# VinAIResearch/GeoFormer

Hardware: AMD Instinct MI355X
Metric: scenes/sec forward (ScanNetV2 ~150k pts) (higher is better)
Workload: dtype f32

## Files before the change

### geoformer_amd/csrc/mask_head.hip

```cpp
#include "common.h"

#ifndef MH_Q
#define MH_Q 2
#endif
#ifndef MH_MINB
#define MH_MINB 3
#endif

__device__ __forceinline__ float mh_xor32(float v, int lane) {
    const auto r = __builtin_amdgcn_permlane32_swap(__float_as_uint(v), __float_as_uint(v), false, false);
    return __uint_as_float(lane < 32 ? r[1] : r[0]);
}
__device__ __forceinline__ float mh_xor16(float v, int lane) {
    const auto r = __builtin_amdgcn_permlane16_swap(__float_as_uint(v), __float_as_uint(v), false, false);
    return __uint_as_float((lane & 16) ? r[0] : r[1]);
}

__device__ __forceinline__ float mh_relu(float x) { return __int_as_float(max(__float_as_int(x), 0)); }

typedef short bf16x4 __attribute__((ext_vector_type(4)));
typedef short mh_s8 __attribute__((ext_vector_type(8)));
typedef __bf16 mh_bf16x8 __attribute__((ext_vector_type(8)));
__device__ __forceinline__ f32x4 mh_mfma2(bf16x4 a1, bf16x4 a2, bf16x4 b1, bf16x4 b2, f32x4 acc) {
    const mh_s8 a = __builtin_shufflevector(a1, a2, 0, 1, 2, 3, 4, 5, 6, 7), b = __builtin_shufflevector(b1, b2, 0, 1, 2, 3, 4, 5, 6, 7);
    return __builtin_amdgcn_mfma_f32_16x16x32_bf16(__builtin_bit_cast(mh_bf16x8, a), __builtin_bit_cast(mh_bf16x8, b), acc, 0, 0, 0);
}
__device__ __forceinline__ void mh_split3(float x, unsigned& h, unsigned& m, unsigned& l) {
    const unsigned hb = __float_as_uint(x) & 0xffff0000u;
    const float r1 = x - __uint_as_float(hb);
    const unsigned mb = __float_as_uint(r1) & 0xffff0000u;
    const float r2 = r1 - __uint_as_float(mb);
    h = hb >> 16;
    m = mb >> 16;
    l = __float_as_uint(r2) >> 16;
}
__device__ __forceinline__ void mh_split3x4(const float (&x)[4], bf16x4& h, bf16x4& m, bf16x4& l) {
#pragma unroll
    for (int s = 0; s < 4; s++) {
        unsigned a, b, c;
        mh_split3(x[s], a, b, c);
        h[s] = (short)a;
        m[s] = (short)b;
        l[s] = (short)c;
    }
}
__global__ void k_mh_split(const float* __restrict__ feat, int n16, unsigned short* __restrict__ fs) {
    const int i = blockIdx.x * blockDim.x + threadIdx.x;
    if (i >= n16) return;
    unsigned h, m, l;
    mh_split3(feat[i], h, m, l);
    fs[i] = (unsigned short)h;
    fs[(size_t)n16 + i] = (unsigned short)m;
    fs[2 * (size_t)n16 + i] = (unsigned short)l;
}

template <bool USE_GEO, bool SPLIT, bool TINY>
__global__ __launch_bounds__(256, MH_MINB) void k_mask_head(const float* __restrict__ feat, const float* __restrict__ coords,
                                                      const float* __restrict__ geo, const float* __restrict__ qxyz,
                                                      const float* __restrict__ mx, const float* __restrict__ w1,
                                                      const float* __restrict__ b1, const float* __restrict__ w2,
                                                      const float* __restrict__ b2, int ldp, int N, int nq, int qmod,
                                                      int chunks, const unsigned short* __restrict__ fs,
                                                      float* __restrict__ out) {
    const int ld_w1 = ldp ? ldp : 16 * 19, ld_v = ldp ? ldp : 16, ld_s = ldp ? ldp : 1;
    const int lane = threadIdx.x & 63, g = lane >> 4, j = lane & 15;
    const int wave = (blockIdx.x * blockDim.x + threadIdx.x) >> 6;
    const int qgroups = (nq + MH_Q - 1) / MH_Q;
    const int qg = wave % qgroups, chunk = wave / qgroups;
    if (chunk >= chunks) return;
    const int nblocks = (N + 63) >> 6;
    const int per = (nblocks + chunks - 1) / chunks;
    const int blk0 = chunk * per, blk1 = min(nblocks, blk0 + per);

    float wf[MH_Q][4];
    float w5[MH_Q];
    float ww[MH_Q][4], b2q[MH_Q], qc[MH_Q], mq[MH_Q];
#pragma unroll
    for (int t = 0; t < MH_Q; t++) {
        const int q = min(qg * MH_Q + t, nq - 1);
        const float* W = w1 + (size_t)q * ld_w1;
#pragma unroll
        for (int s = 0; s < 4; s++) wf[t][s] = W[j * 19 + 3 + 4 * g + s];
        w5[t] = g < 3 ? W[j * 19 + g] : b1[(size_t)q * ld_v + j];
#pragma unroll
        for (int r = 0; r < 4; r++) ww[t][r] = w2[(size_t)q * ld_v + 4 * g + r];
        b2q[t] = b2[(size_t)q * ld_s];
        const int qs = q % qmod;
        qc[t] = g < 3 ? qxyz[qs * 3 + g] : 1.f;
        mq[t] = (USE_GEO && g < 3) ? mx[qs] : 0.f;
    }
    bf16x4 wh[MH_Q], wm[MH_Q], wl[MH_Q];
    if constexpr (SPLIT) {
#pragma unroll
        for (int t = 0; t < MH_Q; t++) mh_split3x4(wf[t], wh[t], wm[t], wl[t]);
    }
    int qrow[MH_Q];
#pragma unroll
    for (int u = 0; u < MH_Q; u++) qrow[u] = min(qg * MH_Q + u, nq - 1) % qmod;

    struct Block {
        float4 f[4];
        bf16x4 fh[4], fm[4], fl[4];
        float pc[4];
        float gd[MH_Q][4];
    };
    const size_t n16 = (size_t)N * 16;
    auto fetch = [&](int blk, Block& B) {
        const int p0 = TINY ? blk * 64 : min(blk * 64, N - 64);
#pragma unroll
        for (int t = 0; t < 4; t++) {
            const int pc = TINY ? min(p0 + 16 * t + j, N - 1) : p0 + 16 * t + j;
            if constexpr (SPLIT) {
                const size_t e = (size_t)pc * 16 + 4 * g;
                B.fh[t] = *reinterpret_cast<const bf16x4*>(fs + e);
                B.fm[t] = *reinterpret_cast<const bf16x4*>(fs + n16 + e);
                B.fl[t] = *reinterpret_cast<const bf16x4*>(fs + 2 * n16 + e);
            } else {
                B.f[t] = *reinterpret_cast<const float4*>(feat + (size_t)pc * 16 + 4 * g);
            }
            B.pc[t] = g < 3 ? coords[(size_t)pc * 3 + g] : 0.f;
#pragma unroll
            for (int u = 0; u < MH_Q; u++)
                B.gd[u][t] = USE_GEO ? geo[(size_t)qrow[u] * N + pc] : 0.f;
        }
    };
    auto compute = [&](const Block& cur, int blk) {
        const int p0 = TINY ? blk * 64 : min(blk * 64, N - 64);
#pragma unroll
        for (int t = 0; t < MH_Q; t++) {
            const int q = qg * MH_Q + t;
            float part[4];
#pragma unroll
            for (int tl = 0; tl < 4; tl++) {
                float rel = qc[t] - cur.pc[tl];
                if (USE_GEO) {
                    const float ms = __uint_as_float((__float_as_uint(rel) & 0x80000000u) | __float_as_uint(mq[t]));
                    rel = rel + ((cur.gd[t][tl] < 0.f && rel != 0.f) ? ms : 0.f);
                }
                f32x4 acc = {0.f, 0.f, 0.f, 0.f};
                acc = __builtin_amdgcn_mfma_f32_16x16x4f32(w5[t], rel, acc, 0, 0, 0);
                if constexpr (SPLIT) {
                    acc = mh_mfma2(wl[t], wh[t], cur.fh[tl], cur.fl[tl], acc);
                    acc = mh_mfma2(wm[t], wm[t], cur.fm[tl], cur.fh[tl], acc);
                    acc = mh_mfma2(wh[t], wh[t], cur.fm[tl], cur.fh[tl], acc);
                } else {
                    acc = __builtin_amdgcn_mfma_f32_16x16x4f32(wf[t][0], cur.f[tl].x, acc, 0, 0, 0);
                    acc = __builtin_amdgcn_mfma_f32_16x16x4f32(wf[t][1], cur.f[tl].y, acc, 0, 0, 0);
                    acc = __builtin_amdgcn_mfma_f32_16x16x4f32(wf[t][2], cur.f[tl].z, acc, 0, 0, 0);
                    acc = __builtin_amdgcn_mfma_f32_16x16x4f32(wf[t][3], cur.f[tl].w, acc, 0, 0, 0);
                }
                float s = 0.f;
#pragma unroll
                for (int r = 0; r < 4; r++) s = fmaf(ww[t][r], mh_relu(acc[r]), s);
                part[tl] = s;
            }
            {
                const bool hi = g >= 2;
                const float send0 = hi ? part[0] : part[2], send1 = hi ? part[1] : part[3];
                const float r0 = mh_xor32(send0, lane), r1 = mh_xor32(send1, lane);
                const float k0 = (hi ? part[2] : part[0]) + r0, k1 = (hi ? part[3] : part[1]) + r1;
                const bool odd = g & 1;
                const float send = odd ? k0 : k1;
                const float r = mh_xor16(send, lane);
                const float tot = (odd ? k1 : k0) + r + b2q[t];
                const int p = p0 + 16 * g + j;
                if (p < N && q < nq) out[(size_t)q * N + p] = tot;
            }
        }
    };
    Block bufA, bufB;
    if (blk0 < blk1) fetch(blk0, bufA);
    for (int blk = blk0; blk < blk1; blk += 2) {
        if (blk + 1 < blk1) fetch(blk + 1, bufB);
        compute(bufA, blk);
        if (blk + 1 < blk1) {
            if (blk + 2 < blk1) fetch(blk + 2, bufA);
            compute(bufB, blk + 1);
        }
    }
}

extern "C" int gf_mask_head_packed(const float* feat, const float* coords, const float* geo, const float* qxyz,
                                   const float* sqrt_max_geo, const float* w1, const float* b1, const float* w2,
                                   const float* b2, int ldp, int N, int nq, int C, float* out, void* stream);
extern "C" int gf_mask_head_episodes(const float* feat, const float* coords, const float* geo, const float* qxyz,
                                     const float* sqrt_max_geo, const float* w1, const float* b1, const float* w2,
                                     const float* b2, int ldp, int N, int nq, int E, int C, void* split_ws, float* out,
                                     void* stream);
extern "C" size_t gf_mask_head_split_bytes(int N) { return (size_t)(N > 0 ? N : 0) * 16 * 3 * sizeof(unsigned short); }
extern "C" int gf_mask_head(const float* feat, const float* coords, const float* geo, const float* qxyz,
                            const float* sqrt_max_geo, const float* w1, const float* b1, const float* w2,
                            const float* b2, int N, int nq, int C, float* out, void* stream) {
    return gf_mask_head_packed(feat, coords, geo, qxyz, sqrt_max_geo, w1, b1, w2, b2, 0, N, nq, C, out, stream);
}

extern "C" int gf_mask_head_packed(const float* feat, const float* coords, const float* geo, const float* qxyz,
                                   const float* sqrt_max_geo, const float* w1, const float* b1, const float* w2,
                                   const float* b2, int ldp, int N, int nq, int C, float* out, void* stream) {
    return gf_mask_head_episodes(feat, coords, geo, qxyz, sqrt_max_geo, w1, b1, w2, b2, ldp, N, nq, 1, C, nullptr, out, stream);
}

extern "C" int gf_mask_head_episodes(const float* feat, const float* coords, const float* geo, const float* qxyz,
                                     const float* sqrt_max_geo, const float* w1, const float* b1, const float* w2,
                                     const float* b2, int ldp, int N, int nq_scene, int E, int C, void* split_ws, float* out,
                                     void* stream) {
    GF_CHECK_ARG(ldp >= 0, "gf_mask_head: negative parameter stride");
    GF_CHECK_ARG(C == 16, "gf_mask_head: only the 16-channel mask head (m=16) is implemented, got C=%d", C);
    GF_CHECK_ARG(N >= 0 && nq_scene >= 0 && E >= 1, "gf_mask_head: bad sizes");
    GF_CHECK_ARG((long long)nq_scene * E < (1ll << 30), "gf_mask_head: %d episodes x %d queries", E, nq_scene);
    GF_CHECK_ARG((geo == nullptr) == (sqrt_max_geo == nullptr), "gf_mask_head: geo and sqrt_max_geo come together");
    if (N == 0 || nq_scene == 0) return GF_OK;
    const int qmod = nq_scene, nq = nq_scene * E;
    const int qgroups = (nq + MH_Q - 1) / MH_Q;
    const int nblocks = (N + 63) / 64;
    int chunks = (256 * 4 * 8 + qgroups - 1) / qgroups;
    if (chunks > nblocks) chunks = nblocks;
    if (chunks < 1) chunks = 1;
    const long long waves = (long long)qgroups * chunks;
    dim3 grid((unsigned)((waves + 3) / 4));
    hipStream_t st = (hipStream_t)stream;
    const unsigned short* fs = (const unsigned short*)split_ws;
    if (fs) {
        GF_CHECK_ARG(((uintptr_t)fs % 8) == 0, "gf_mask_head: split_ws must be 8-byte aligned");
        const int n16 = N * 16;
        hipLaunchKernelGGL(k_mh_split, dim3(gf_div_up(n16, 256)), dim3(256), 0, st, feat, n16, (unsigned short*)split_ws);
    }
#define MH_LAUNCH(GEO_, SPLIT_)                                                                                          \
    do {                                                                                                                 \
        if (N < 64)                                                                                                      \
            GF_LAUNCH_OP(GF_OP_MASK_HEAD, (k_mask_head<GEO_, SPLIT_, true>), grid, dim3(256), 0, st, feat, coords, geo, qxyz, \
                         sqrt_max_geo, w1, b1, w2, b2, ldp, N, nq, qmod, chunks, fs, out);                               \
        else                                                                                                             \
            GF_LAUNCH_OP(GF_OP_MASK_HEAD, (k_mask_head<GEO_, SPLIT_, false>), grid, dim3(256), 0, st, feat, coords, geo, qxyz, \
                         sqrt_max_geo, w1, b1, w2, b2, ldp, N, nq, qmod, chunks, fs, out);                               \
    } while (0)
    if (geo && fs) MH_LAUNCH(true, true);
    else if (geo) MH_LAUNCH(true, false);
    else if (fs) MH_LAUNCH(false, true);
    else MH_LAUNCH(false, false);
#undef MH_LAUNCH
    GF_CHECK_LAUNCH("gf_mask_head");
    return GF_OK;
}

#define MHB_Q 4

template <bool USE_GEO>
__global__ __launch_bounds__(256, 2) void k_mask_head_bwd_feat(const float* __restrict__ feat, const float* __restrict__ coords,
                                                               const float* __restrict__ geo, const float* __restrict__ qxyz,
                                                               const float* __restrict__ mx, const float* __restrict__ w1,
                                                               const float* __restrict__ b1, const float* __restrict__ w2,
                                                               const float* __restrict__ gout, int ldp, int N, int nq,
                                                               int qmod, int qsplit, float* __restrict__ dfeat) {
    const int ld_w1 = ldp ? ldp : 16 * 19, ld_v = ldp ? ldp : 16;
    const int lane = threadIdx.x & 63, g = lane >> 4, j = lane & 15;
    const int wave = (blockIdx.x * blockDim.x + threadIdx.x) >> 6;
    const int nblocks = (N + 63) >> 6;
    const int blk = wave / qsplit, part = wave - blk * qsplit;
// ... 255 lines not shown
```

### geoformer_amd/model/geoformer.py

```python
from __future__ import annotations

import functools
import os

import numpy as np
import torch
import torch.nn as nn
from torch.nn import functional as F

from .. import _lib, pointops, spconv, unet_exec, unet_train
from . import config as _config
from .backbone import ResidualBlock, UBlock, conv1d_bn_relu, random_downsample
from .layers import (BatchNorm1d, BigLinear, GenericMLP, LazyRelPos, PointwiseConv1d, PositionEmbeddingCoordsSine, RelPosSpec,
                     TransformerDecoder,
                     TransformerDecoderLayer, scene_counts)
from .set_abstraction import PointnetSAModuleVotesSeparate


class _Voxelization(torch.autograd.Function):

    @staticmethod
    def forward(ctx, feats, map_rule, mode=4):
        ctx.rule, ctx.mode, ctx.N = map_rule, mode, feats.shape[0]
        return pointops.voxelize_fp(feats.contiguous(), map_rule, mode)
# ... 800 lines not shown
    def mask_heads_forward(self, geo_dist, mask_features, weights, biases, num_insts, coords_, fps_sampling_coords,
                           use_geo=True):
        n_mask = mask_features.size(0)
        if (mask_features.is_cuda and self.output_dim == 16 and not torch.is_grad_enabled()):
            mx = None
            if use_geo:
                early = self._early()
                hit = next((early.pop(k) for k in list(early) if k[0] == "mx" and early[k][0] is geo_dist), None)
                if hit is not None:
                    torch.cuda.current_stream().wait_event(hit[2])
                    mx = hit[1]
                else:
                    mx = torch.max(geo_dist, dim=1)[0]
                    mx = torch.sqrt(torch.where(mx < 0, torch.max(mx), mx)).contiguous()
            od = self.output_dim
            logits = pointops.mask_head(
                mask_features.reshape(n_mask, od).contiguous(), coords_.contiguous(),
                geo_dist.contiguous() if use_geo else None, fps_sampling_coords.reshape(-1, 3).contiguous(), mx,
                weights[0].reshape(num_insts, od, od + 3).contiguous(), biases[0].reshape(num_insts, od).contiguous(),
                weights[1].reshape(num_insts, od).contiguous(), biases[1].reshape(num_insts).contiguous())
            return logits.reshape(1, num_insts, n_mask)
        rel = fps_sampling_coords.reshape(-1, 1, 3) - coords_.reshape(1, -1, 3)
        if use_geo:
            mx = torch.max(geo_dist, dim=1)[0]
            mx = torch.sqrt(torch.where(mx < 0, torch.max(mx), mx))
            rel = torch.where((geo_dist < 0).unsqueeze(-1), rel + mx[:, None, None] * torch.sign(rel), rel)
        w1, w2 = weights[0].reshape(num_insts, self.output_dim, -1), weights[1].reshape(num_insts, 1, -1)
        b1, b2 = biases[0].reshape(num_insts, self.output_dim, 1), biases[1].reshape(num_insts, 1, 1)
        feat = mask_features.reshape(n_mask, -1)
        h = torch.matmul(w1[:, :, :3], rel.permute(0, 2, 1)) + torch.matmul(w1[:, :, 3:], feat.t().unsqueeze(0)) + b1
        x = torch.matmul(w2, F.relu(h)) + b2
        return x.reshape(1, num_insts, n_mask)

    def _mask_head_packed(self, geo_dist, mask_features, params, num_insts, coords_, fps_sampling_coords):
        n_mask = mask_features.size(0)
        early = self._early()
        hit = next((early.pop(k) for k in list(early) if k[0] == "mx" and early[k][0] is geo_dist), None)
        if hit is not None:
            torch.cuda.current_stream().wait_event(hit[2])
            mx = hit[1]
        else:
            mx = torch.max(geo_dist, dim=1)[0]
            mx = torch.sqrt(torch.where(mx < 0, torch.max(mx), mx)).contiguous()
        logits = pointops.mask_head_packed(mask_features.reshape(n_mask, self.output_dim).contiguous(),
                                           coords_.contiguous(), geo_dist.contiguous(),
                                           fps_sampling_coords.reshape(-1, 3).contiguous(), mx, params.contiguous())
        return logits.reshape(1, num_insts, n_mask)

    def get_mask_prediction(self, geo_dists, param_kernels, mask_features, locs_float_, fps_sampling_locs,
                            batch_offsets_):
        num_layers, n_queries, batch = param_kernels.shape[:3]
        offs = _offsets_list(batch_offsets_)
        outputs = []
        fused_train = (mask_features.is_cuda and torch.is_grad_enabled() and self.output_dim == 16 and self.use_coords
                       and os.environ.get("GF_FUSED_BWD", "1") != "0")
        per_scene, train_ctrl = {}, {}
        if fused_train:
            for b in range(batch):
                s, e = offs[b], offs[b + 1]
                if e - s == 0:
                    continue
                g = geo_dists[b].contiguous()
                mx = torch.max(g, dim=1)[0]
                mx = torch.sqrt(torch.where(mx < 0, torch.max(mx), mx)).contiguous()
                per_scene[b] = (mask_features[s:e].reshape(e - s, self.output_dim).contiguous(),
                                locs_float_[s:e].contiguous(), g, fps_sampling_locs[b].reshape(-1, 3).contiguous(), mx)
        for l, pk in enumerate(param_kernels.unbind(0) if fused_train else param_kernels):
            pk2 = pk.transpose(0, 1).flatten(0, 1)
            sem_chain = self._pointwise_chain("detr_sem_head", [self.detr_sem_head], pk2)
            tow_chain = self._pointwise_chain("before_embedding_tower", [self.before_embedding_tower], pk2)
            packed = False
            if sem_chain is not None and tow_chain is not None:
                rows = pk2.contiguous()
                packed = self.output_dim == 16 and self.use_coords
                cls_done = None
                if packed and rows.is_cuda and not torch.is_grad_enabled() and batch == 1 and not pointops.co_resident():
                    main = torch.cuda.current_stream(rows.device)
                    aux = _SIDE_STREAMS.get((rows.device, main.cuda_stream, "aux"))
                    if aux is not None:
                        rows_ready = torch.cuda.Event()
                        rows_ready.record(main)
                        aux.wait_event(rows_ready)
                        with torch.cuda.stream(aux):
                            cls_logits = pointops.pointwise_mlp(rows, sem_chain).reshape(batch, n_queries, -1)
                            cls_done = torch.cuda.Event()
                            cls_done.record(aux)
                        rows.record_stream(aux)
                        cls_logits.record_stream(main)
                if cls_done is None:
                    cls_logits = pointops.pointwise_mlp(rows, sem_chain).reshape(batch, n_queries, -1)
                emb = pointops.pointwise_mlp(rows, tow_chain)
                controllers = F.linear(emb, self.controller.weight[:, :, 0], self.controller.bias)
            else:
                cls_logits = self.detr_sem_head(pk.permute(1, 2, 0)).transpose(1, 2)
                controllers = self.controller(self.before_embedding_tower(pk2.unsqueeze(2))).squeeze(2)
            controllers = controllers.reshape(batch, n_queries, -1)
            ctrl = controllers.unbind(0) if fused_train else controllers
            mask_logits_list = []
            for b in range(batch):
                s, e = offs[b], offs[b + 1]
                if e - s == 0:
                    mask_logits_list.append(None)
                    continue
                if packed and mask_features.is_cuda and not torch.is_grad_enabled():
                    ml = self._mask_head_packed(geo_dists[b], mask_features[s:e], controllers[b], n_queries,
                                                locs_float_[s:e], fps_sampling_locs[b])
                elif fused_train:
                    train_ctrl.setdefault(b, []).append(ctrl[b])
                    mask_logits_list.append(None)
                    continue
                else:
                    weights, biases = self.parse_dynamic_params(controllers[b], self.output_dim)
                    ml = self.mask_heads_forward(geo_dists[b], mask_features[s:e], weights, biases, n_queries,
                                                 locs_float_[s:e], fps_sampling_locs[b], use_geo=self.use_coords)
                mask_logits_list.append(ml.squeeze(0))
            if packed and cls_done is not None:
                torch.cuda.current_stream(cls_logits.device).wait_event(cls_done)
            outputs.append({"cls_logits": cls_logits, "mask_logits": mask_logits_list})
        for b, ctrls in train_ctrl.items():
            mf_b, locs_b, g, fps_b, mx = per_scene[b]
            logits = pointops.mask_head_train_episodes(mf_b, torch.stack(ctrls), locs_b, g, fps_b, mx)
            for l, ml in enumerate(logits.unbind(0)):
                outputs[l]["mask_logits"][b] = ml
        return outputs

    def generate_proposal(self, mask_logits, cls_logits, fg_idxs, batch_offsets, batch_offsets_,
                          semantic_scores_=None, logit_thresh=0.5, score_thresh=0.5, npoint_thresh=100, sem_prob=None,
                          defer=False, knn_flags=(), segments=None):
        b = 0
        segments = None if torch.is_grad_enabled() else _segments_arg(segments)
        if mask_logits[b].is_cuda and not torch.is_grad_enabled():
            offs, offs_ = _offsets_list(batch_offsets), _offsets_list(batch_offsets_)
            num_points = int(offs[b + 1] - offs[b])
            logits = mask_logits[b].contiguous()
            if sem_prob is not None and isinstance(sem_prob, tuple):
                sem_t = sem_prob[1][:, offs_[b]:offs_[b + 1]]
            else:
                sem = sem_prob if sem_prob is not None else F.softmax(semantic_scores_, dim=1)
                sem_t = sem[offs_[b]:offs_[b + 1]].t()
# ... 152 lines not shown
        if len(fg_idxs) == 0:
            if agree is not None:
                agree(False, locs_float.device)
            outputs["mask_predictions"] = None
            if all_scenes:
                empty = [([], [], []) for _ in range(batch_size)]
                outputs["proposal_scores_per_scene"] = PendingBatchProposals(batch_size, value=empty) \
                    if defer_proposals else empty
            return outputs
        if not fused_fg:
            batch_idxs_ = batch_idxs[fg_idxs]
            locs_float_ = locs_float[fg_idxs]
            output_feats_ = pointops.take_rows_unique(output_feats, fg_idxs)
            semantic_scores_ = semantic_scores[fg_idxs]
        batch_offsets_ = get_batch_offsets(batch_idxs_, batch_size, host_only=fused_fg and not training)
        offs_ = _offsets_list(batch_offsets_)
        nonempty = min(offs_[b + 1] - offs_[b] for b in range(batch_size)) > 0
        n_scenes, scene_ids = batch_size, list(range(batch_size))
        if all_scenes and not nonempty:
            scene_ids = [b for b in range(batch_size) if offs_[b + 1] > offs_[b]]
            offs_ = [offs_[b] for b in scene_ids] + [offs_[-1]]
            batch_offsets_ = torch.tensor(offs_, dtype=torch.int32, device=batch_offsets_.device)
            pc_dims = [pc_dims[0][scene_ids], pc_dims[1][scene_ids]]
            batch_size, nonempty = len(scene_ids), True
        if agree is not None and not agree(nonempty, locs_float.device):
            outputs["mask_predictions"] = None
            return outputs

        def sampling_independent(graphs_only=None):
            if graphs_only is True:
                return knn_graphs(locs_float_, batch_offsets_, batch_size, neighbor=64, radius=0.05)
            chain = self._pointwise_chain("mask_tower", [self.mask_tower], output_feats_)
            if chain is not None:
                mf = pointops.pointwise_mlp(output_feats_.contiguous(), chain).unsqueeze(2)
            else:
                mf = self._mask_tower_rows(output_feats_)
                if mf is None:
                    mf = self.mask_tower(output_feats_.unsqueeze(2).permute(2, 1, 0)).permute(2, 1, 0)
            sp = None
            if not training:
                sp = F.softmax(semantic_scores_, dim=1)
                if sp.is_cuda:
                    sp = (sp, sp.t().contiguous())
            if graphs_only is False:
                return mf, sp
            gr = None
            if locs_float_.is_cuda and nonempty:
                gr = knn_graphs(locs_float_, batch_offsets_, batch_size, neighbor=64, radius=0.05)
            return mf, sp, gr

        max_step = 128 if self.training else 256
        geo_dists = None
        overlap = locs_float_.is_cuda and nonempty and os.environ.get("GF_OVERLAP", "1") != "0"
        if overlap and fused_fg and not training:
            contexts, geo_dists, (mask_features_, sem_prob, graphs) = self._aggregate_geodesic_overlapped(
                locs_float_, output_feats_, batch_offsets_, batch_size, None, max_step, pc_dims, epilogue=True,
                early=sampling_independent, presampled=presampled if fused_fg else None,
                presampled_before=draw_bufs["before"] if (fused_fg and presampled is not None) else None)
        else:
            mask_features_, sem_prob, graphs = sampling_independent()
            if graphs is not None and overlap:
                contexts, geo_dists = self._aggregate_geodesic_overlapped(locs_float_, output_feats_, batch_offsets_,
                                                                          batch_size, graphs, max_step, pc_dims,
                                                                          epilogue=not torch.is_grad_enabled())
            else:
                contexts = self.forward_aggregator(locs_float_, output_feats_, batch_offsets_, batch_size)
        if contexts is None:
# ... 61 lines not shown
```

### geoformer_amd/pointops.py

```python
from __future__ import annotations

import contextlib
import os
import threading

import numpy as np
import torch

from . import _abi, _lib
from ._lib import check, ptr, stream_ptr


def _f32c(t, name):
    if not (t.is_cuda and t.dtype == torch.float32 and t.is_contiguous()):
        raise RuntimeError(f"{name}: expected a contiguous float32 tensor on the GPU")
    return t


def _i32c(t, name):
    if not (t.is_cuda and t.dtype == torch.int32 and t.is_contiguous()):
        raise RuntimeError(f"{name}: expected a contiguous int32 tensor on the GPU")
    return t


# ... 341 lines not shown
        dev = torch.device(device)
        idx = dev.index if dev.index is not None else torch.cuda.current_device()
    for key in list(_SCRATCH):
        if device is None or key[0] == idx:
            del _SCRATCH[key]


def scratch_bytes():
    return sum(t.numel() * t.element_size() for t in _SCRATCH.values() if t is not None)


def geodesic_bfs(D, I, deg, src, radius, max_step, wg_threads=1024):
    _f32c(D, "D"); _i32c(I, "I"); _i32c(src, "src")
    n, K = D.shape
    nq = src.shape[0]
    dev = D.device
    geo = torch.empty((nq, n), dtype=torch.float32, device=dev)
    lib = _lib.load()
    keys = scratch("bfs_keys", nq * n, torch.int64, dev)
    qwords = int(lib.gf_geodesic_bfs_queue_words(n))
    queues = scratch("bfs_queues", nq * qwords, torch.int32, dev)
    check(lib.gf_geodesic_bfs_cfg(ptr(D), ptr(I), ptr(deg), n, K, ptr(src), nq, float(radius), int(max_step),
                                          ptr(geo), ptr(keys), ptr(queues), qwords, int(wg_threads), stream_ptr()),
          "gf_geodesic_bfs")
    return geo


def _mask_head_split_ws(N, device, split):
    if not split:
        return None
    return scratch("mask_head_split", _lib.load().gf_mask_head_split_bytes(N) // 8 + 1, torch.int64, device)


def mask_head(feat, coords, geo, qxyz, sqrt_max_geo, w1, b1, w2, b2, split=True):
    for t, name in ((feat, "feat"), (coords, "coords"), (qxyz, "qxyz"), (w1, "w1"), (b1, "b1"), (w2, "w2"), (b2, "b2")):
        _f32c(t, name)
    N, C = feat.shape
    nq = qxyz.shape[0]
    out = torch.empty((nq, N), dtype=torch.float32, device=feat.device)
    check(_lib.load().gf_mask_head_episodes(ptr(feat), ptr(coords), ptr(geo), ptr(qxyz), ptr(sqrt_max_geo), ptr(w1), ptr(b1),
                                            ptr(w2), ptr(b2), 0, N, nq, 1, C, ptr(_mask_head_split_ws(N, feat.device, split)),
                                            ptr(out), stream_ptr()), "gf_mask_head")
    return out


def mask_head_packed(feat, coords, geo, qxyz, sqrt_max_geo, params, split=True):
    return mask_head_episodes(feat, coords, geo, qxyz, sqrt_max_geo, params.unsqueeze(0), split=split)[0]


def mask_head_episodes(feat, coords, geo, qxyz, sqrt_max_geo, params, split=True):
    for t, name in ((feat, "feat"), (coords, "coords"), (qxyz, "qxyz"), (params, "params")):
        _f32c(t, name)
    N, C = feat.shape
    E, nq, ld = params.shape
    if ld != C * (C + 3) + C + C + 1 or qxyz.shape[0] != nq:
        raise RuntimeError(f"mask_head_episodes: params {tuple(params.shape)} for {qxyz.shape[0]} queries, C={C}")
    base = params.data_ptr()
    o_w2, o_b1, o_b2 = C * (C + 3), C * (C + 3) + C, C * (C + 3) + 2 * C
    out = torch.empty((E, nq, N), dtype=torch.float32, device=feat.device)
    check(_lib.load().gf_mask_head_episodes(ptr(feat), ptr(coords), ptr(geo), ptr(qxyz), ptr(sqrt_max_geo), base,
                                            base + 4 * o_b1, base + 4 * o_w2, base + 4 * o_b2, ld, N, nq, E, C,
                                            ptr(_mask_head_split_ws(N, feat.device, split)), ptr(out), stream_ptr()),
          "gf_mask_head_episodes")
    return out


class _MaskHeadFn(torch.autograd.Function):

    @staticmethod
    def forward(ctx, feat, params, coords, geo, qxyz, sqrt_max_geo):
        ctx.save_for_backward(feat, params, coords, geo, qxyz, sqrt_max_geo)
        return mask_head_packed(feat, coords, geo, qxyz, sqrt_max_geo, params)

    @staticmethod
    def backward(ctx, gout):
        feat, params, coords, geo, qxyz, mx = ctx.saved_tensors
        N, C = feat.shape
        nq, ld = params.shape
        lib = _lib.load()
        dparams = torch.empty_like(params)
        dfeat = torch.zeros_like(feat)
        scratch = torch.empty(lib.gf_mask_head_bwd_scratch_floats(N, nq), dtype=torch.float32, device=feat.device)
        base = params.data_ptr()
        o_w2, o_b1 = C * (C + 3), C * (C + 3) + C
        check(lib.gf_mask_head_bwd(ptr(feat), ptr(coords), ptr(geo), ptr(qxyz), ptr(mx), base, base + 4 * o_b1,
                                   base + 4 * o_w2, ptr(gout.contiguous()), ld, N, nq, C, ptr(dparams), ptr(dfeat),
                                   ptr(scratch), stream_ptr()), "gf_mask_head_bwd")
        return dfeat, dparams, None, None, None, None


class _MaskHeadEpisodesFn(torch.autograd.Function):

    @staticmethod
    def forward(ctx, feat, params, coords, geo, qxyz, sqrt_max_geo):
        ctx.save_for_backward(feat, params, coords, geo, qxyz, sqrt_max_geo)
# ... 1421 lines not shown
```

### include/geoformer_hip.h

```cpp
#ifndef GEOFORMER_HIP_H
#define GEOFORMER_HIP_H

#include <stddef.h>
#include <stdint.h>

#ifdef __cplusplus
extern "C" {
#endif

#define GF_ABI_VERSION 7

typedef enum {
    GF_OK = 0,
    GF_ERR_INVALID_ARG = -1,
    GF_ERR_LAUNCH = -2,
    GF_ERR_UNSUPPORTED = -3,
    GF_ERR_CALLBACK = -4,
} gf_status;

int gf_abi_version(void);
const char* gf_last_error(void);

size_t gf_fg_scratch_bytes(int N);
int gf_fg_select(const float* scores, int N, int C, int cls, int mode, const float* locs, const int32_t* batch_idxs,
// ... 192 lines not shown
int gf_group_points_grad(const float* grad_out, const int32_t* idx, int b, int c, int n, int npoints, int nsample,
                         float* grad_points, void* stream);
int gf_ball_query(const float* new_xyz, const float* xyz, int b, int n, int m, float radius, int nsample, int32_t* idx,
                  void* stream);
size_t gf_fps_scratch_bytes(int b);
int gf_furthest_point_sampling(const float* xyz, int b, int n, int m, int32_t* idxs, void* scratch, void* stream);
const int32_t* gf_fps_error_flag(void* scratch, int b);
int gf_furthest_point_sampling_resume(const float* xyz, int b, int n, int m, int m_known, int32_t* idxs,
                                      void* scratch, void* stream);


size_t gf_knn_scratch_bytes(int n);
int gf_knn_radius(const float* xyz, int n, int k, float radius, int sqrt_out, float* D, int32_t* I, int32_t* deg,
                  void* scratch, void* stream);
const int32_t* gf_knn_error_flag(void* scratch, int n);

size_t gf_geodesic_bfs_queue_words(int n);
int gf_geodesic_bfs(const float* D, const int32_t* I, const int32_t* deg, int n, int K, const int32_t* src, int nq,
                    float radius, int max_step, float* geo, void* keys_ws, void* queue_ws, void* stream);
int gf_geodesic_bfs_cfg(const float* D, const int32_t* I, const int32_t* deg, int n, int K, const int32_t* src, int nq,
                        float radius, int max_step, float* geo, void* keys_ws, void* queue_ws, size_t queue_words,
                        int wg_threads, void* stream);

int gf_mask_head(const float* feat, const float* coords, const float* geo, const float* qxyz,
                 const float* sqrt_max_geo, const float* w1, const float* b1, const float* w2, const float* b2, int N,
                 int nq, int C, float* out, void* stream);
int gf_mask_head_packed(const float* feat, const float* coords, const float* geo, const float* qxyz,
                        const float* sqrt_max_geo, const float* w1, const float* b1, const float* w2, const float* b2,
                        int ldp, int N, int nq, int C, float* out, void* stream);
size_t gf_mask_head_split_bytes(int N);
int gf_mask_head_episodes(const float* feat, const float* coords, const float* geo, const float* qxyz,
                          const float* sqrt_max_geo, const float* w1, const float* b1, const float* w2, const float* b2,
                          int ldp, int N, int nq, int E, int C, void* split_ws, float* out, void* stream);

size_t gf_mask_head_bwd_scratch_floats(int N, int nq);
int gf_mask_head_bwd(const float* feat, const float* coords, const float* geo, const float* qxyz,
                     const float* sqrt_max_geo, const float* w1, const float* b1, const float* w2, const float* gout,
                     int ldp, int N, int nq, int C, float* dparams, float* dfeat, float* scratch, void* stream);
int gf_mask_head_bwd_episodes(const float* feat, const float* coords, const float* geo, const float* qxyz,
                              const float* sqrt_max_geo, const float* w1, const float* b1, const float* w2,
                              const float* gout, int ldp, int N, int nq, int E, int C, float* dparams, float* dfeat,
                              float* scratch, void* stream);


int gf_pointwise_mlp(const float* x, int N, int n_layers, const float* const* W, const float* const* scale,
                     const float* const* shift, const int* channels, const int* relu, float* out, void* stream);
int gf_pointwise_mlp_rows(const float* x, const int32_t* rows, int N, int n_layers, const float* const* W,
                          const float* const* scale, const float* const* shift, const int* channels, const int* relu,
                          float* out, void* stream);

int gf_group_mlp_max(const float* grouped, int B, int npoint, int nsample, int n_layers, const float* const* W,
                     const float* const* scale, const float* const* shift, const int* channels, const int* relu,
                     float* out, void* stream);

int gf_ball_query_centres(const float* xyz, const int32_t* centre_idx, int b, int n, int m, float radius, int nsample,
                          float* new_xyz, int32_t* idx, void* stream);
int gf_point_grid_build(const float* xyz, int n, float radius, void* scratch, void* stream);
int gf_ball_query_grid(const float* xyz, int n, const int32_t* centre_idx, const float* centres, int m, float radius,
                       int nsample, void* scratch, int grid_ready, float* new_xyz, int32_t* idx, void* stream);
int gf_sa_group_mlp_max(const float* xyz, const float* feats, const int32_t* inds, int B, int n, int C, int npoint,
                        float radius, int nsample, int use_xyz, int normalize_xyz, int n_layers,
                        const float* const* W, const float* const* scale, const float* const* shift,
                        const int* channels, const int* relu, float* new_xyz, int32_t* idx, float* out, void* scratch,
                        int grid_ready, void* stream);

int gf_softmax_dim1_fwd(const float* x, int n0, int n1, int inner, float scale, float* y, void* stream);
// ... 467 lines not shown
```

Measured before the change: 227.4.

## Interleave mask-head bf16 split layout, use buffer loads, and precompute split once

The bf16 hi/mid/lo split of the mask features is now stored interleaved per 4-channel group, so each lane fetches its operands with two 128-bit buffer loads instead of three 64-bit loads. The pre-shuffled weight operands feed the bf16 MFMAs directly. Addressing moves to buffer resources with scalar base offsets, and the output reduction uses paired permlane swaps followed by a buffer store. The split is computed right after the mask tower and reused by the mask head when the tensor version matches, which removes the per-call split kernel. This adds a 2^24-point limit and a Python-side cache tied to tensor versions.

```diff
diff --git a/geoformer_amd/csrc/mask_head.hip b/geoformer_amd/csrc/mask_head.hip
--- a/geoformer_amd/csrc/mask_head.hip
+++ b/geoformer_amd/csrc/mask_head.hip
@@ -1,4 +1,5 @@
 #include "common.h"
+#include "conv_tile.h"
 
 #ifndef MH_Q
 #define MH_Q 2
@@ -18,13 +19,15 @@
 
 __device__ __forceinline__ float mh_relu(float x) { return __int_as_float(max(__float_as_int(x), 0)); }
 
+__device__ __forceinline__ const float* mh_uniform(const float* p) {
+    const unsigned long long a = (unsigned long long)p;
+    const unsigned lo = __builtin_amdgcn_readfirstlane((unsigned)a), hi = __builtin_amdgcn_readfirstlane((unsigned)(a >> 32));
+    return (const float*)(((unsigned long long)hi << 32) | lo);
+}
+
 typedef short bf16x4 __attribute__((ext_vector_type(4)));
 typedef short mh_s8 __attribute__((ext_vector_type(8)));
 typedef __bf16 mh_bf16x8 __attribute__((ext_vector_type(8)));
-__device__ __forceinline__ f32x4 mh_mfma2(bf16x4 a1, bf16x4 a2, bf16x4 b1, bf16x4 b2, f32x4 acc) {
-    const mh_s8 a = __builtin_shufflevector(a1, a2, 0, 1, 2, 3, 4, 5, 6, 7), b = __builtin_shufflevector(b1, b2, 0, 1, 2, 3, 4, 5, 6, 7);
-    return __builtin_amdgcn_mfma_f32_16x16x32_bf16(__builtin_bit_cast(mh_bf16x8, a), __builtin_bit_cast(mh_bf16x8, b), acc, 0, 0, 0);
-}
 __device__ __forceinline__ void mh_split3(float x, unsigned& h, unsigned& m, unsigned& l) {
     const unsigned hb = __float_as_uint(x) & 0xffff0000u;
     const float r1 = x - __uint_as_float(hb);
@@ -44,14 +47,16 @@
         l[s] = (short)c;
     }
 }
-__global__ void k_mh_split(const float* __restrict__ feat, int n16, unsigned short* __restrict__ fs) {
+__global__ void k_mh_split(const float4* __restrict__ feat4, int n4, bf16x4* __restrict__ fs) {
     const int i = blockIdx.x * blockDim.x + threadIdx.x;
-    if (i >= n16) return;
-    unsigned h, m, l;
-    mh_split3(feat[i], h, m, l);
-    fs[i] = (unsigned short)h;
-    fs[(size_t)n16 + i] = (unsigned short)m;
-    fs[2 * (size_t)n16 + i] = (unsigned short)l;
+    if (i >= n4) return;
+    const float4 v = feat4[i];
+    const float x[4] = {v.x, v.y, v.z, v.w};
+    bf16x4 h, m, l;
+    mh_split3x4(x, h, m, l);
+    fs[3 * (size_t)i] = m;
+    fs[3 * (size_t)i + 1] = h;
+    fs[3 * (size_t)i + 2] = l;
 }
 
 template <bool USE_GEO, bool SPLIT, bool TINY>
@@ -64,7 +69,7 @@
                                                       float* __restrict__ out) {
     const int ld_w1 = ldp ? ldp : 16 * 19, ld_v = ldp ? ldp : 16, ld_s = ldp ? ldp : 1;
     const int lane = threadIdx.x & 63, g = lane >> 4, j = lane & 15;
-    const int wave = (blockIdx.x * blockDim.x + threadIdx.x) >> 6;
+    const int wave = blockIdx.x * 4 + __builtin_amdgcn_readfirstlane(threadIdx.x >> 6);
     const int qgroups = (nq + MH_Q - 1) / MH_Q;
     const int qg = wave % qgroups, chunk = wave / qgroups;
     if (chunk >= chunks) return;
@@ -89,82 +94,98 @@
         qc[t] = g < 3 ? qxyz[qs * 3 + g] : 1.f;
         mq[t] = (USE_GEO && g < 3) ? mx[qs] : 0.f;
     }
-    bf16x4 wh[MH_Q], wm[MH_Q], wl[MH_Q];
+    mh_bf16x8 a_lh[MH_Q], a_mm[MH_Q], a_hh[MH_Q];
     if constexpr (SPLIT) {
 #pragma unroll
-        for (int t = 0; t < MH_Q; t++) mh_split3x4(wf[t], wh[t], wm[t], wl[t]);
-    }
-    int qrow[MH_Q];
-#pragma unroll
-    for (int u = 0; u < MH_Q; u++) qrow[u] = min(qg * MH_Q + u, nq - 1) % qmod;
+        for (int t = 0; t < MH_Q; t++) {
+            bf16x4 wh, wm, wl;
+            mh_split3x4(wf[t], wh, wm, wl);
+            a_lh[t] = __builtin_bit_cast(mh_bf16x8, (mh_s8)__builtin_shufflevector(wl, wh, 0, 1, 2, 3, 4, 5, 6, 7));
+            a_mm[t] = __builtin_bit_cast(mh_bf16x8, (mh_s8)__builtin_shufflevector(wm, wm, 0, 1, 2, 3, 4, 5, 6, 7));
+            a_hh[t] = __builtin_bit_cast(mh_bf16x8, (mh_s8)__builtin_shufflevector(wh, wh, 0, 1, 2, 3, 4, 5, 6, 7));
+        }
+    }
+
+    constexpr unsigned FP = SPLIT ? 96u : 64u;
+    const __amdgpu_buffer_rsrc_t rs_f = gf_buffer_rsrc(SPLIT ? (const void*)fs : (const void*)feat, N * (int)FP);
+    const __amdgpu_buffer_rsrc_t rs_c = gf_buffer_rsrc(coords, N * 12);
+    __amdgpu_buffer_rsrc_t rs_g[MH_Q], rs_o[MH_Q];
+#pragma unroll
+    for (int u = 0; u < MH_Q; u++) {
+        const int q = min(qg * MH_Q + u, nq - 1);
+        rs_g[u] = gf_buffer_rsrc(USE_GEO ? mh_uniform(geo + (size_t)(q % qmod) * N) : nullptr, USE_GEO ? N * 4 : 0);
+        rs_o[u] = gf_buffer_rsrc(mh_uniform(out + (size_t)q * N), N * 4);
+    }
+    const unsigned fo = j * FP + g * (FP / 4), co = g < 3 ? j * 12u + g * 4u : 0x80000000u, go = j * 4u, oo = lane * 4u;
 
     struct Block {
-        float4 f[4];
-        bf16x4 fh[4], fm[4], fl[4];
+        u32x4 f[4];
+        u32x4 fb[4];
         float pc[4];
         float gd[MH_Q][4];
     };
-    const size_t n16 = (size_t)N * 16;
+    auto first_point = [&](int blk) { return (unsigned)(TINY ? blk * 64 : min(blk * 64, N - 64)); };
     auto fetch = [&](int blk, Block& B) {
-        const int p0 = TINY ? blk * 64 : min(blk * 64, N - 64);
+        const unsigned p0 = first_point(blk);
 #pragma unroll
         for (int t = 0; t < 4; t++) {
-            const int pc = TINY ? min(p0 + 16 * t + j, N - 1) : p0 + 16 * t + j;
-            if constexpr (SPLIT) {
-                const size_t e = (size_t)pc * 16 + 4 * g;
-                B.fh[t] = *reinterpret_cast<const bf16x4*>(fs + e);
-                B.fm[t] = *reinterpret_cast<const bf16x4*>(fs + n16 + e);
-                B.fl[t] = *reinterpret_cast<const bf16x4*>(fs + 2 * n16 + e);
-            } else {
-                B.f[t] = *reinterpret_cast<const float4*>(feat + (size_t)pc * 16 + 4 * g);
-            }
-            B.pc[t] = g < 3 ? coords[(size_t)pc * 3 + g] : 0.f;
+            B.f[t] = __builtin_amdgcn_raw_buffer_load_b128(rs_f, fo + t * 16u * FP, p0 * FP, 0);
+            if constexpr (SPLIT) B.fb[t] = __builtin_amdgcn_raw_buffer_load_b128(rs_f, fo + t * 16u * FP + 8u, p0 * FP, 0);
+            B.pc[t] = __uint_as_float(__builtin_amdgcn_raw_buffer_load_b32(rs_c, co + t * 192u, p0 * 12u, 0));
 #pragma unroll
             for (int u = 0; u < MH_Q; u++)
-                B.gd[u][t] = USE_GEO ? geo[(size_t)qrow[u] * N + pc] : 0.f;
+                B.gd[u][t] = USE_GEO ? __uint_as_float(__builtin_amdgcn_raw_buffer_load_b32(rs_g[u], go + t * 64u, p0 * 4u, 0)) : 0.f;
         }
     };
     auto compute = [&](const Block& cur, int blk) {
-        const int p0 = TINY ? blk * 64 : min(blk * 64, N - 64);
+        const unsigned p0 = first_point(blk);
 #pragma unroll
         for (int t = 0; t < MH_Q; t++) {
             const int q = qg * MH_Q + t;
             float part[4];
 #pragma unroll
-            for (int tl = 0; tl < 4; tl++) {
-                float rel = qc[t] - cur.pc[tl];
-                if (USE_GEO) {
-                    const float ms = __uint_as_float((__float_as_uint(rel) & 0x80000000u) | __float_as_uint(mq[t]));
-                    rel = rel + ((cur.gd[t][tl] < 0.f && rel != 0.f) ? ms : 0.f);
+            for (int tp = 0; tp < 2; tp++) {
+                f32x4 acc2[2];
+#pragma unroll
+                for (int h = 0; h < 2; h++) {
+                    const int tl = 2 * tp + h;
+                    float rel = qc[t] - cur.pc[tl];
+                    if (USE_GEO) {
+                        const float ms = __uint_as_float((__float_as_uint(rel) & 0x80000000u) | __float_as_uint(mq[t]));
+                        rel = rel + ((cur.gd[t][tl] < 0.f && rel != 0.f) ? ms : 0.f);
+                    }
+                    f32x4 acc = {0.f, 0.f, 0.f, 0.f};
+                    acc = __builtin_amdgcn_mfma_f32_16x16x4f32(w5[t], rel, acc, 0, 0, 0);
+                    if constexpr (SPLIT) {
+                        const mh_bf16x8 f_mh = __builtin_bit_cast(mh_bf16x8, cur.f[tl]), f_hl = __builtin_bit_cast(mh_bf16x8, cur.fb[tl]);
+                        acc = __builtin_amdgcn_mfma_f32_16x16x32_bf16(a_lh[t], f_hl, acc, 0, 0, 0);
+                        acc = __builtin_amdgcn_mfma_f32_16x16x32_bf16(a_mm[t], f_mh, acc, 0, 0, 0);
+                        acc = __builtin_amdgcn_mfma_f32_16x16x32_bf16(a_hh[t], f_mh, acc, 0, 0, 0);
+                    } else {
+                        const float4 f = gf_as_float4(cur.f[tl]);
+                        acc = __builtin_amdgcn_mfma_f32_16x16x4f32(wf[t][0], f.x, acc, 0, 0, 0);
+                        acc = __builtin_amdgcn_mfma_f32_16x16x4f32(wf[t][1], f.y, acc, 0, 0, 0);
+                        acc = __builtin_amdgcn_mfma_f32_16x16x4f32(wf[t][2], f.z, acc, 0, 0, 0);
+                        acc = __builtin_amdgcn_mfma_f32_16x16x4f32(wf[t][3], f.w, acc, 0, 0, 0);
+                    }
+                    acc2[h] = acc;
                 }
-                f32x4 acc = {0.f, 0.f, 0.f, 0.f};
-                acc = __builtin_amdgcn_mfma_f32_16x16x4f32(w5[t], rel, acc, 0, 0, 0);
-                if constexpr (SPLIT) {
-                    acc = mh_mfma2(wl[t], wh[t], cur.fh[tl], cur.fl[tl], acc);
-                    acc = mh_mfma2(wm[t], wm[t], cur.fm[tl], cur.fh[tl], acc);
-                    acc = mh_mfma2(wh[t], wh[t], cur.fm[tl], cur.fh[tl], acc);
-                } else {
-                    acc = __builtin_amdgcn_mfma_f32_16x16x4f32(wf[t][0], cur.f[tl].x, acc, 0, 0, 0);
-                    acc = __builtin_amdgcn_mfma_f32_16x16x4f32(wf[t][1], cur.f[tl].y, acc, 0, 0, 0);
-                    acc = __builtin_amdgcn_mfma_f32_16x16x4f32(wf[t][2], cur.f[tl].z, acc, 0, 0, 0);
-                    acc = __builtin_amdgcn_mfma_f32_16x16x4f32(wf[t][3], cur.f[tl].w, acc, 0, 0, 0);
+                float sa = 0.f, sb = 0.f;
+#pragma unroll
+                for (int r = 0; r < 4; r++) {
+                    sa = fmaf(ww[t][r], mh_relu(acc2[0][r]), sa);
+                    sb = fmaf(ww[t][r], mh_relu(acc2[1][r]), sb);
                 }
-                float s = 0.f;
-#pragma unroll
-                for (int r = 0; r < 4; r++) s = fmaf(ww[t][r], mh_relu(acc[r]), s);
-                part[tl] = s;
+                part[2 * tp] = sa;
+                part[2 * tp + 1] = sb;
             }
             {
-                const bool hi = g >= 2;
-                const float send0 = hi ? part[0] : part[2], send1 = hi ? part[1] : part[3];
-                const float r0 = mh_xor32(send0, lane), r1 = mh_xor32(send1, lane);
-                const float k0 = (hi ? part[2] : part[0]) + r0, k1 = (hi ? part[3] : part[1]) + r1;
-                const bool odd = g & 1;
-                const float send = odd ? k0 : k1;
-                const float r = mh_xor16(send, lane);
-                const float tot = (odd ? k1 : k0) + r + b2q[t];
-                const int p = p0 + 16 * g + j;
-                if (p < N && q < nq) out[(size_t)q * N + p] = tot;
+                const auto s0 = __builtin_amdgcn_permlane32_swap(__float_as_uint(part[0]), __float_as_uint(part[2]), false, false);
+                const auto s1 = __builtin_amdgcn_permlane32_swap(__float_as_uint(part[1]), __float_as_uint(part[3]), false, false);
+                const float k0 = __uint_as_float(s0[0]) + __uint_as_float(s0[1]), k1 = __uint_as_float(s1[0]) + __uint_as_float(s1[1]);
+                const auto s2 = __builtin_amdgcn_permlane16_swap(__float_as_uint(k0), __float_as_uint(k1), false, false);
+                const float tot = __uint_as_float(s2[0]) + __uint_as_float(s2[1]) + b2q[t];
+                if (q < nq) __builtin_amdgcn_raw_buffer_store_b32(__float_as_uint(tot), rs_o[t], oo, p0 * 4u, 0);
             }
         }
     };
@@ -187,7 +208,23 @@
                                      const float* sqrt_max_geo, const float* w1, const float* b1, const float* w2,
                                      const float* b2, int ldp, int N, int nq, int E, int C, void* split_ws, float* out,
                                      void* stream);
+extern "C" int gf_mask_head_episodes_ws(const float* feat, const float* coords, const float* geo, const float* qxyz,
+                                        const float* sqrt_max_geo, const float* w1, const float* b1, const float* w2,
+                                        const float* b2, int ldp, int N, int nq, int E, int C, void* split_ws, int split_filled,
+                                        float* out, void* stream);
 extern "C" size_t gf_mask_head_split_bytes(int N) { return (size_t)(N > 0 ? N : 0) * 16 * 3 * sizeof(unsigned short); }
+
+extern "C" int gf_mask_head_split(const float* feat, int N, int C, void* split_ws, void* stream) {
+    GF_CHECK_ARG(C == 16, "gf_mask_head_split: only the 16-channel mask head (m=16) is implemented, got C=%d", C);
+    GF_CHECK_ARG(N >= 0 && N <= (1 << 24), "gf_mask_head_split: %d points", N);
+    GF_CHECK_ARG(split_ws && ((uintptr_t)split_ws % 8) == 0, "gf_mask_head_split: split_ws must be 8-byte aligned");
+    if (N == 0) return GF_OK;
+    const int n4 = N * 4;
+    hipLaunchKernelGGL(k_mh_split, dim3(gf_div_up(n4, 256)), dim3(256), 0, (hipStream_t)stream, (const float4*)feat, n4,
+                       (bf16x4*)split_ws);
+    GF_CHECK_LAUNCH("gf_mask_head_split");
+    return GF_OK;
+}
 extern "C" int gf_mask_head(const float* feat, const float* coords, const float* geo, const float* qxyz,
                             const float* sqrt_max_geo, const float* w1, const float* b1, const float* w2,
                             const float* b2, int N, int nq, int C, float* out, void* stream) {
@@ -204,11 +241,21 @@
                                      const float* sqrt_max_geo, const float* w1, const float* b1, const float* w2,
                                      const float* b2, int ldp, int N, int nq_scene, int E, int C, void* split_ws, float* out,
                                      void* stream) {
+    return gf_mask_head_episodes_ws(feat, coords, geo, qxyz, sqrt_max_geo, w1, b1, w2, b2, ldp, N, nq_scene, E, C, split_ws, 0,
+                                    out, stream);
+}
+
+extern "C" int gf_mask_head_episodes_ws(const float* feat, const float* coords, const float* geo, const float* qxyz,
+                                        const float* sqrt_max_geo, const float* w1, const float* b1, const float* w2,
+                                        const float* b2, int ldp, int N, int nq_scene, int E, int C, void* split_ws,
+                                        int split_filled, float* out, void* stream) {
     GF_CHECK_ARG(ldp >= 0, "gf_mask_head: negative parameter stride");
     GF_CHECK_ARG(C == 16, "gf_mask_head: only the 16-channel mask head (m=16) is implemented, got C=%d", C);
     GF_CHECK_ARG(N >= 0 && nq_scene >= 0 && E >= 1, "gf_mask_head: bad sizes");
     GF_CHECK_ARG((long long)nq_scene * E < (1ll << 30), "gf_mask_head: %d episodes x %d queries", E, nq_scene);
+    GF_CHECK_ARG(N <= (1 << 24), "gf_mask_head: %d points (the kernel addresses a scene with 32-bit byte offsets)", N);
     GF_CHECK_ARG((geo == nullptr) == (sqrt_max_geo == nullptr), "gf_mask_head: geo and sqrt_max_geo come together");
+    GF_CHECK_ARG(!split_filled || split_ws, "gf_mask_head: split_filled without split_ws");
     if (N == 0 || nq_scene == 0) return GF_OK;
     const int qmod = nq_scene, nq = nq_scene * E;
     const int qgroups = (nq + MH_Q - 1) / MH_Q;
@@ -222,8 +269,10 @@
     const unsigned short* fs = (const unsigned short*)split_ws;
     if (fs) {
         GF_CHECK_ARG(((uintptr_t)fs % 8) == 0, "gf_mask_head: split_ws must be 8-byte aligned");
-        const int n16 = N * 16;
-        hipLaunchKernelGGL(k_mh_split, dim3(gf_div_up(n16, 256)), dim3(256), 0, st, feat, n16, (unsigned short*)split_ws);
+        if (!split_filled) {
+            const int n4 = N * 4;
+            hipLaunchKernelGGL(k_mh_split, dim3(gf_div_up(n4, 256)), dim3(256), 0, st, (const float4*)feat, n4, (bf16x4*)split_ws);
+        }
     }
 #define MH_LAUNCH(GEO_, SPLIT_)                                                                                          \
     do {                                                                                                                 \
diff --git a/geoformer_amd/model/geoformer.py b/geoformer_amd/model/geoformer.py
--- a/geoformer_amd/model/geoformer.py
+++ b/geoformer_amd/model/geoformer.py
@@ -856,7 +856,7 @@
         x = torch.matmul(w2, F.relu(h)) + b2
         return x.reshape(1, num_insts, n_mask)
 
-    def _mask_head_packed(self, geo_dist, mask_features, params, num_insts, coords_, fps_sampling_coords):
+    def _mask_head_packed(self, geo_dist, mask_features, params, num_insts, coords_, fps_sampling_coords, split_ws=None):
         n_mask = mask_features.size(0)
         early = self._early()
         hit = next((early.pop(k) for k in list(early) if k[0] == "mx" and early[k][0] is geo_dist), None)
@@ -868,7 +868,8 @@
             mx = torch.sqrt(torch.where(mx < 0, torch.max(mx), mx)).contiguous()
         logits = pointops.mask_head_packed(mask_features.reshape(n_mask, self.output_dim).contiguous(),
                                            coords_.contiguous(), geo_dist.contiguous(),
-                                           fps_sampling_coords.reshape(-1, 3).contiguous(), mx, params.contiguous())
+                                           fps_sampling_coords.reshape(-1, 3).contiguous(), mx, params.contiguous(),
+                                           split_ws=split_ws)
         return logits.reshape(1, num_insts, n_mask)
 
     def get_mask_prediction(self, geo_dists, param_kernels, mask_features, locs_float_, fps_sampling_locs,
@@ -927,8 +928,14 @@
                     mask_logits_list.append(None)
                     continue
                 if packed and mask_features.is_cuda and not torch.is_grad_enabled():
+                    ws = None
+                    ahead = getattr(mask_features, "_gf_split", None)
+                    if (ahead is not None and batch == 1 and s == 0 and e == ahead[0].shape[0]
+                            and ahead[0].data_ptr() == mask_features.data_ptr() and ahead[0]._version == ahead[1]):
+                        ws = ahead[2]
+                        ws.record_stream(torch.cuda.current_stream(ws.device))
                     ml = self._mask_head_packed(geo_dists[b], mask_features[s:e], controllers[b], n_queries,
-                                                locs_float_[s:e], fps_sampling_locs[b])
+                                                locs_float_[s:e], fps_sampling_locs[b], split_ws=ws)
                 elif fused_train:
                     train_ctrl.setdefault(b, []).append(ctrl[b])
                     mask_logits_list.append(None)
@@ -1147,7 +1154,11 @@
                 return knn_graphs(locs_float_, batch_offsets_, batch_size, neighbor=64, radius=0.05)
             chain = self._pointwise_chain("mask_tower", [self.mask_tower], output_feats_)
             if chain is not None:
-                mf = pointops.pointwise_mlp(output_feats_.contiguous(), chain).unsqueeze(2)
+                rows = pointops.pointwise_mlp(output_feats_.contiguous(), chain)
+                mf = rows.unsqueeze(2)
+                if (not training and batch_size == 1 and rows.is_cuda and self.output_dim == 16 and self.use_coords
+                        and not torch.is_grad_enabled()):
+                    mf._gf_split = (rows, rows._version, pointops.mask_head_split(rows))
             else:
                 mf = self._mask_tower_rows(output_feats_)
                 if mf is None:
diff --git a/geoformer_amd/pointops.py b/geoformer_amd/pointops.py
--- a/geoformer_amd/pointops.py
+++ b/geoformer_amd/pointops.py
@@ -397,23 +397,44 @@
     return scratch("mask_head_split", _lib.load().gf_mask_head_split_bytes(N) // 8 + 1, torch.int64, device)
 
 
-def mask_head(feat, coords, geo, qxyz, sqrt_max_geo, w1, b1, w2, b2, split=True):
+def mask_head_split(feat):
+    _f32c(feat, "feat")
+    N, C = feat.shape
+    lib = _lib.load()
+    ws = torch.empty(lib.gf_mask_head_split_bytes(N) // 8 + 1, dtype=torch.int64, device=feat.device)
+    check(lib.gf_mask_head_split(ptr(feat), N, C, ptr(ws), stream_ptr()), "gf_mask_head_split")
+    return ws
+
+
+def _mask_head_ws(N, device, split, split_ws):
+    if split_ws is None:
+        return _mask_head_split_ws(N, device, split), 0
+    if not split:
+        raise RuntimeError("mask_head: split_ws with split=False")
+    if split_ws.dtype != torch.int64 or split_ws.device != device or \
+            split_ws.numel() * 8 < _lib.load().gf_mask_head_split_bytes(N):
+        raise RuntimeError(f"mask_head: split_ws is not mask_head_split() of {N} points on {device}")
+    return split_ws, 1
+
+
+def mask_head(feat, coords, geo, qxyz, sqrt_max_geo, w1, b1, w2, b2, split=True, split_ws=None):
     for t, name in ((feat, "feat"), (coords, "coords"), (qxyz, "qxyz"), (w1, "w1"), (b1, "b1"), (w2, "w2"), (b2, "b2")):
         _f32c(t, name)
     N, C = feat.shape
     nq = qxyz.shape[0]
     out = torch.empty((nq, N), dtype=torch.float32, device=feat.device)
-    check(_lib.load().gf_mask_head_episodes(ptr(feat), ptr(coords), ptr(geo), ptr(qxyz), ptr(sqrt_max_geo), ptr(w1), ptr(b1),
-                                            ptr(w2), ptr(b2), 0, N, nq, 1, C, ptr(_mask_head_split_ws(N, feat.device, split)),
-                                            ptr(out), stream_ptr()), "gf_mask_head")
+    ws, filled = _mask_head_ws(N, feat.device, split, split_ws)
+    check(_lib.load().gf_mask_head_episodes_ws(ptr(feat), ptr(coords), ptr(geo), ptr(qxyz), ptr(sqrt_max_geo), ptr(w1),
+                                               ptr(b1), ptr(w2), ptr(b2), 0, N, nq, 1, C, ptr(ws), filled, ptr(out),
+                                               stream_ptr()), "gf_mask_head")
     return out
 
 
-def mask_head_packed(feat, coords, geo, qxyz, sqrt_max_geo, params, split=True):
-    return mask_head_episodes(feat, coords, geo, qxyz, sqrt_max_geo, params.unsqueeze(0), split=split)[0]
-
-
-def mask_head_episodes(feat, coords, geo, qxyz, sqrt_max_geo, params, split=True):
+def mask_head_packed(feat, coords, geo, qxyz, sqrt_max_geo, params, split=True, split_ws=None):
+    return mask_head_episodes(feat, coords, geo, qxyz, sqrt_max_geo, params.unsqueeze(0), split=split, split_ws=split_ws)[0]
+
+
+def mask_head_episodes(feat, coords, geo, qxyz, sqrt_max_geo, params, split=True, split_ws=None):
     for t, name in ((feat, "feat"), (coords, "coords"), (qxyz, "qxyz"), (params, "params")):
         _f32c(t, name)
     N, C = feat.shape
@@ -423,9 +444,10 @@
     base = params.data_ptr()
     o_w2, o_b1, o_b2 = C * (C + 3), C * (C + 3) + C, C * (C + 3) + 2 * C
     out = torch.empty((E, nq, N), dtype=torch.float32, device=feat.device)
-    check(_lib.load().gf_mask_head_episodes(ptr(feat), ptr(coords), ptr(geo), ptr(qxyz), ptr(sqrt_max_geo), base,
-                                            base + 4 * o_b1, base + 4 * o_w2, base + 4 * o_b2, ld, N, nq, E, C,
-                                            ptr(_mask_head_split_ws(N, feat.device, split)), ptr(out), stream_ptr()),
+    ws, filled = _mask_head_ws(N, feat.device, split, split_ws)
+    check(_lib.load().gf_mask_head_episodes_ws(ptr(feat), ptr(coords), ptr(geo), ptr(qxyz), ptr(sqrt_max_geo), base,
+                                               base + 4 * o_b1, base + 4 * o_w2, base + 4 * o_b2, ld, N, nq, E, C,
+                                               ptr(ws), filled, ptr(out), stream_ptr()),
           "gf_mask_head_episodes")
     return out
 
diff --git a/include/geoformer_hip.h b/include/geoformer_hip.h
--- a/include/geoformer_hip.h
+++ b/include/geoformer_hip.h
@@ -248,6 +248,11 @@
 int gf_mask_head_episodes(const float* feat, const float* coords, const float* geo, const float* qxyz,
                           const float* sqrt_max_geo, const float* w1, const float* b1, const float* w2, const float* b2,
                           int ldp, int N, int nq, int E, int C, void* split_ws, float* out, void* stream);
+int gf_mask_head_split(const float* feat, int N, int C, void* split_ws, void* stream);
+int gf_mask_head_episodes_ws(const float* feat, const float* coords, const float* geo, const float* qxyz,
+                             const float* sqrt_max_geo, const float* w1, const float* b1, const float* w2, const float* b2,
+                             int ldp, int N, int nq, int E, int C, void* split_ws, int split_filled, float* out,
+                             void* stream);
 
 size_t gf_mask_head_bwd_scratch_floats(int N, int nq);
 int gf_mask_head_bwd(const float* feat, const float* coords, const float* geo, const float* qxyz,
```

After: 224.1. 1.4% lower.
